# Lumina-Group/libzkp

Hardware: AMD Instinct MI355X
Metric: proofs/sec (whole node) + ms/proof p50, 4096-proof mixed batch (range / equality / membership / improvement) per MI355X (higher is better)
Workload: dtype u32/u64 integer limbs (10x25.5-bit GF(2^255-19), BN254 Fq on 9x29-bit limbs in the MSM loops and 10x26-bit elsewhere, 8x32-bit Fr and scalars mod l, 2x64-bit f128)

## Files before the change

### libzkp_amd/csrc/g16_circuit.h

```cpp
#pragma once
#include <mutex>
#include <array>
#include <map>
#include <vector>
#include <cstring>
#include "g16_steps.h"
#include "sha256_host.h"

namespace zkp {

inline fr fr_pow_words(fr base, const uint32_t e[8]) {
    fr acc = fp_one<FrParams>();
    for (int i = 255; i >= 0; i--) { acc = fp_sq(acc); if ((e[i >> 5] >> (i & 31)) & 1u) acc = fp_mul(acc, base); }
    return acc;
}
inline void put_fr(std::vector<uint32_t>& v, const fr& x) { for (int k = 0; k < 8; k++) v.push_back(x.v[k]); }

struct HostLC { std::map<uint32_t, fr> t; };
struct HostR1CS {
    uint32_t n_inst = 1, n_wit = 0;
    std::vector<std::array<HostLC, 3>> rows;
    std::vector<uint8_t> inst_nwin{1}, wit_nwin;
    uint32_t new_input(uint8_t nwin) { inst_nwin.push_back(nwin); return n_inst++; }
    uint32_t new_witness(uint8_t nwin) { wit_nwin.push_back(nwin); return 0x80000000u | n_wit++; }
// ... 18 lines not shown
}
inline void r1cs_enforce_equal(HostR1CS& cs, const HostLC& a, const HostLC& b) { cs.rows.push_back({lc_sub(a, b), lc_var(VAR_ONE), HostLC{}}); }

inline std::vector<fr> g_mimc_host;
inline std::once_flag g_mimc_once;
inline void ensure_mimc_constants() {
    std::call_once(g_mimc_once, []() {
        for (uint32_t i = 0; i < MIMC_ROUNDS; i++) {
            uint8_t in[23]; memcpy(in, "libzkp_mimc_v1:", 15); for (int k = 0; k < 8; k++) in[15 + k] = (uint8_t)((uint64_t)i >> (8 * k));
            uint8_t h[32]; sha256_host(h, in, 23);
            uint32_t w[8]; memcpy(w, h, 32);
            g_mimc_host.push_back(fp_from_raw<FrParams>(w));
        }
    });
}
inline HostLC r1cs_mimc(HostR1CS& cs, HostLC x) {
    ensure_mimc_constants();
    for (uint32_t i = 0; i < MIMC_ROUNDS; i++) {
        const HostLC t = lc_add(x, lc_scale(lc_var(VAR_ONE), g_mimc_host[i]));
        const uint32_t t2 = r1cs_mul(cs, t, t, G16_NW_FULL);
        const uint32_t t4 = r1cs_mul(cs, lc_var(t2), lc_var(t2), G16_NW_FULL);
        x = lc_var(r1cs_mul(cs, lc_var(t4), t, G16_NW_FULL));
    }
    return x;
}
inline HostR1CS build_equality_r1cs() {
    HostR1CS cs;
    const uint32_t a = cs.new_witness(G16_NW_U64), b = cs.new_witness(G16_NW_U64);
    r1cs_enforce_equal(cs, lc_var(a), lc_var(b));
    const HostLC h = r1cs_mimc(cs, lc_var(a));
    const uint32_t c = cs.new_input(G16_NW_FULL);
    r1cs_enforce_equal(cs, h, lc_var(c));
    return cs;
}
inline HostR1CS build_membership_r1cs() {
    HostR1CS cs;
    const uint32_t v = cs.new_witness(G16_NW_U64);
    const HostLC h = r1cs_mimc(cs, lc_var(v));
    const uint32_t c = cs.new_input(G16_NW_FULL);
    r1cs_enforce_equal(cs, h, lc_var(c));
    std::vector<uint32_t> setv, real, sel;
    for (uint32_t i = 0; i < G16_MAX_SET; i++) setv.push_back(cs.new_input(G16_NW_U64));
    for (uint32_t i = 0; i < G16_MAX_SET; i++) { const uint32_t b = cs.new_input(1); cs.rows.push_back({lc_sub(lc_var(VAR_ONE), lc_var(b)), lc_var(b), HostLC{}}); real.push_back(b); }
    for (uint32_t i = 0; i < G16_MAX_SET; i++) { const uint32_t b = cs.new_witness(1); cs.rows.push_back({lc_sub(lc_var(VAR_ONE), lc_var(b)), lc_var(b), HostLC{}}); sel.push_back(b); }
    HostLC total;
    for (uint32_t i = 0; i < G16_MAX_SET; i++) {
        total = lc_add(total, lc_var(sel[i]));
        const uint32_t p = r1cs_mul(cs, lc_var(sel[i]), lc_sub(lc_var(VAR_ONE), lc_var(real[i])), 1);
        r1cs_enforce_equal(cs, lc_var(p), HostLC{});
    }
    r1cs_enforce_equal(cs, total, lc_var(VAR_ONE));
    HostLC acc;
    for (uint32_t i = 0; i < G16_MAX_SET; i++) acc = lc_add(acc, lc_var(r1cs_mul(cs, lc_var(sel[i]), lc_sub(lc_var(v), lc_var(setv[i])), G16_NW_FULL)));
    r1cs_enforce_equal(cs, acc, HostLC{});
    return cs;
}


struct HostCircuitTables {
    uint32_t n_inst, n_wit, nv, n_rows, m, logm;
    std::vector<uint32_t> ptr[3], col[3], coef[3];
    std::vector<uint32_t> tw, tw_inv, coset, coset_inv, zinv;
};
inline HostCircuitTables build_circuit_tables(const HostR1CS& cs) {
    HostCircuitTables T;
    T.n_inst = cs.n_inst; T.n_wit = cs.n_wit; T.nv = cs.n_inst + cs.n_wit; T.n_rows = (uint32_t)cs.rows.size();
    uint32_t m = 1, lg = 0; while (m < T.n_rows + T.n_inst) { m <<= 1; lg++; }
    T.m = m; T.logm = lg;
    auto colidx = [&](uint32_t v) { return (v & WIT) ? cs.n_inst + (v & ~WIT) : v; };
    for (int q = 0; q < 3; q++) {
        T.ptr[q].push_back(0);
        for (auto& row : cs.rows) {
            for (auto& kv : row[q].t) { T.col[q].push_back(colidx(kv.first)); put_fr(T.coef[q], kv.second); }
            T.ptr[q].push_back((uint32_t)T.col[q].size());
        }
    }
    uint32_t e[8]; for (int i = 0; i < 8; i++) e[i] = FrParams::mod(i);
    e[0] -= 1;
    for (uint32_t s = 0; s < lg; s++) { for (int i = 0; i < 7; i++) e[i] = (e[i] >> 1) | (e[i + 1] << 31); e[7] >>= 1; }
    const fr g = fp_from_u64<FrParams>(5), w = fr_pow_words(g, e);
    const fr winv = fp_inv(w), ginv = fp_inv(g), minv = fp_inv(fp_from_u64<FrParams>(m));
    auto put_fr9 = [](std::vector<uint32_t>& v, const fr& x) { const fr9 y = fr9_from_fr(x); for (int i = 0; i < 9; i++) v.push_back(y.v[i]); };
    fr a = fp_one<FrParams>(), b = a;
    for (uint32_t j = 0; j < m / 2; j++) { put_fr9(T.tw, a); put_fr9(T.tw_inv, b); a = fp_mul(a, w); b = fp_mul(b, winv); }
    a = minv; b = minv;
    for (uint32_t i = 0; i < m; i++) { put_fr9(T.coset, a); put_fr9(T.coset_inv, b); a = fp_mul(a, g); b = fp_mul(b, ginv); }
    fr gm = fp_one<FrParams>(); for (uint32_t i = 0; i < m; i++) gm = fp_mul(gm, g);
    put_fr9(T.zinv, fp_inv(fp_sub(gm, fp_one<FrParams>())));
    return T;
}

}
```

### libzkp_amd/csrc/g16_impl.inc

```

namespace {

struct G16Key {
    bool loaded = false;
    uint32_t n_inst = 0, n_wit = 0, nv = 0, n_rows = 0, m = 0, logm = 0;
    G16Circuit C{};
    std::vector<void*> allocs;
    uint32_t *table_g1 = nullptr, *table_g2 = nullptr;
    G16Radix rx = g16_radix(G16_WBITS_DEFAULT);
    int shared_tables = -1;
    uint64_t table_bytes = 0;
    struct Chunking { DevLayout lay; const uint32_t* corr = nullptr; const uint16_t* scal = nullptr; };
    std::vector<SlotList> targets_g1, targets_g2;
    std::vector<uint16_t> hscal_g1, hscal_g2;
    std::map<uint64_t, Chunking> lays_g1, lays_g2;
    uint64_t win_g1 = 0, win_g2 = 0;
    const uint32_t *init_g1 = nullptr, *init_g2 = nullptr;
    G16Vk vk{}; bool vk_ready = false;
    const uint32_t *vm_kconst = nullptr, *vm_lines = nullptr;
};
struct G16Run {
    void* buf = nullptr; size_t cap = 0; hipStream_t side = nullptr, side2 = nullptr; hipEvent_t ev[4] = {nullptr, nullptr, nullptr, nullptr};
    hipEvent_t last = nullptr; bool used = false;
};
// ... 348 lines not shown
            uint32_t* d_ic_tab = nullptr;
            if ((rc = build_tables<20>(K, ic_pts, &d_ic_tab, false, g16_radix(G16V_WBITS)))) return rc;
            K.vk.gamma = gamma_g2.p; K.vk.delta = delta_g2.p; K.vk.beta = beta_g2.p; K.vk.n_ic = (uint32_t)abc.size(); K.vk.ic = d_ic; K.vk.ic_table = d_ic_tab;
            K.vk.ml_alpha_beta = miller_loop(beta_g2.p, aff_neg(alpha_g1.p));
            std::vector<uint32_t> kc(6 * 20), lines;
            g16_vm_key_constants(beta_g2.p, aff_neg(alpha_g1.p), gamma_g2.p, delta_g2.p, kc.data(), lines);
            if ((rc = dev_upload(K, &K.vm_kconst, kc)) || (rc = dev_upload(K, &K.vm_lines, lines))) return rc;
            K.vk_ready = true;
        }
    }
    K.loaded = true;
    return 0;
}


fr tape_fr(const uint32_t seed[8], uint32_t idx, uint32_t slot) { uint32_t w[16]; tape_draw64(w, seed, idx, slot); return fp_from_wide<FrParams>(w); }

int gpu_scalar_mults(bool g2, const std::vector<fr>& scalars, std::vector<uint8_t>& out_bytes) {
    const uint32_t rows = (uint32_t)scalars.size(), AW = g2 ? 40 : 20, JW = g2 ? G2_JAC_W : G1_JAC_W, PB = g2 ? 128 : 64;
    std::vector<uint32_t> base;
    if (!g2) append_words(base, host_g1_generator()); else append_words(base, host_g2_generator());
    ensure_offsets();
    std::vector<uint32_t> offs;
    if (!g2) { append_words(offs, g_off.o1); append_words(offs, jac_neg(g_off.o1)); } else { append_words(offs, g_off.o2); append_words(offs, jac_neg(g_off.o2)); }
    const G16Radix rx = g16_radix(10);
    std::vector<uint32_t> dig((size_t)rx.digw * rows);
    for (uint32_t i = 0; i < rows; i++) {
        sc raw; fp_to_raw(raw.v, scalars[i]); uint32_t pk[G16_DIGW_MAX]; g16_recode(pk, raw, rx);
        for (uint32_t k = 0; k < rx.digw; k++) dig[(size_t)k * rows + i] = pk[k];
    }
    uint32_t *d_base = nullptr, *d_tab = nullptr, *d_dig = nullptr, *d_part = nullptr, *d_offs = nullptr, *d_sums = nullptr; uint8_t* d_out = nullptr;
    uint16_t* d_meta = nullptr; uint8_t* d_nwin = nullptr; uint32_t* d_steps = nullptr;
    DevScope mem;
    HIP_TRY(mem.alloc(&d_base, AW * 4)); HIP_TRY(mem.alloc(&d_tab, (size_t)rx.slot_ent * g16_table_entry_words(g2, true) * 4 + 64)); HIP_TRY(mem.alloc(&d_dig, dig.size() * 4));
    HIP_TRY(mem.alloc(&d_part, (size_t)JW * 4 * rows)); HIP_TRY(mem.alloc(&d_sums, (size_t)JW * 4 * rows)); HIP_TRY(mem.alloc(&d_offs, offs.size() * 4));
    HIP_TRY(hipMemcpy(d_offs, offs.data(), offs.size() * 4, hipMemcpyHostToDevice)); HIP_TRY(mem.alloc(&d_out, (size_t)PB * rows)); HIP_TRY(mem.alloc(&d_meta, 32)); HIP_TRY(mem.alloc(&d_nwin, 16));
    const uint16_t meta[7] = {0, 0, 0, 0, (uint16_t)rx.nwin, 0, 1};
    const uint8_t nwin = (uint8_t)rx.nwin;
    HIP_TRY(hipMemcpy(d_base, base.data(), AW * 4, hipMemcpyHostToDevice));
    HIP_TRY(hipMemcpy(d_dig, dig.data(), dig.size() * 4, hipMemcpyHostToDevice));
    HIP_TRY(hipMemcpy(d_meta, meta, 14, hipMemcpyHostToDevice)); HIP_TRY(hipMemcpy(d_nwin, &nwin, 1, hipMemcpyHostToDevice));
    uint32_t steps_words = 0;
    {
        MsmLayout L1; L1.slot_base = {0}; L1.slot_nwin = {(uint8_t)rx.nwin}; L1.chunk_begin = {0}; L1.chunk_win0 = {0}; L1.chunk_nwin = {(uint16_t)rx.nwin}; L1.target_chunk_begin = {0, 1};
        std::vector<uint32_t> steps, step0;
        const GatherShape shape{rx.nent, rx.slot_ent, rx.uneven ? 1u : 0u, rx.digw};
        if (!make_gather_steps(L1, nullptr, shape, steps, step0)) return fail(ZKP_HIP_E_UNSUPPORTED, "window tables of more than 2^32 entries");
        steps.insert(steps.end(), step0.begin(), step0.end());
        HIP_TRY(mem.alloc(&d_steps, steps.size() * 4));
        HIP_TRY(hipMemcpy(d_steps, steps.data(), steps.size() * 4, hipMemcpyHostToDevice));
        steps_words = (uint32_t)(steps.size() - step0.size());
    }
    g16_launch_build_table(g2, d_base, 1, d_tab, dev().stream, true, rx);
    MsmView m; m.nwin = rx.nwin; m.nent = rx.nent; m.digw = rx.digw; m.slot_ent = rx.slot_ent; m.uneven = rx.uneven; m.rows = rows; m.nslots = 1; m.nchunks = 1; m.table = d_tab; m.digits = d_dig;
    m.slot_base = d_meta; m.slot_scalar = d_meta + 1; m.slot_nwin = d_nwin; m.chunk_begin = d_meta + 2; m.chunk_win0 = d_meta + 3; m.chunk_nwin = d_meta + 4; m.partial = d_part; m.acc_init = d_offs;
    m.steps = d_steps; m.chunk_step0 = d_steps + steps_words;
    g16_launch_msm(g2, m, dev().stream);
    ReduceView R{}; R.rows = rows; R.ntargets = 1; R.partial = d_part; R.target_chunk_begin = d_meta + 5; R.corr = d_offs + JW;
    g16_launch_sum(g2, R, d_sums, dev().stream);
    g16_launch_serialize(g2, d_sums, rows, d_out, dev().stream);
    out_bytes.resize((size_t)PB * rows);
    HIP_TRY(hipMemcpyAsync(out_bytes.data(), d_out, out_bytes.size(), hipMemcpyDeviceToHost, dev().stream));
    HIP_TRY(hipStreamSynchronize(dev().stream));
    return 0;
}

int generate_key_locked(int kind, const uint8_t* setup_seed, std::vector<uint8_t>& pk, std::vector<uint8_t>& vk) {
    if (kind != G16_EQUALITY && kind != G16_MEMBERSHIP) return fail(ZKP_HIP_E_ARGUMENT, "unknown circuit kind");
    const HostR1CS cs = kind == G16_EQUALITY ? build_equality_r1cs() : build_membership_r1cs();
    const HostCircuitTables T = build_circuit_tables(cs);
    uint32_t seed[8];
    if (setup_seed) memcpy(seed, setup_seed, 32);
    else { std::vector<uint8_t> f; int rc0 = fresh_seeds(f, 1); if (rc0) return rc0; memcpy(seed, f.data(), 32); }
    const char* tagname = kind == G16_EQUALITY ? "equality_mimc" : "membership_mimc";
    uint8_t th[32]; sha256_host(th, (const uint8_t*)tagname, strlen(tagname));
    const uint32_t tag = (uint32_t)th[0] | ((uint32_t)th[1] << 8) | ((uint32_t)th[2] << 16);
    fr tw[5];
    for (uint32_t k = 0; k < 5; k++) { tw[k] = tape_fr(seed, 0x47313601u, 8 * tag + k); if (fp_is_zero(tw[k])) tw[k] = fp_one<FrParams>(); }
    const fr alpha = tw[0], beta = tw[1], gamma = tw[2], delta = tw[3], tau = tw[4];
    const uint32_t m = T.m, nv = T.nv;
    const fr one = fp_one<FrParams>();
    fr taum = one; for (uint32_t i = 0; i < m; i++) taum = fp_mul(taum, tau);
    const fr zt = fp_sub(taum, one), minv = fp_inv(fp_from_u64<FrParams>(m));
    const fr w = fr9_to_fr<FrParams>(ld_fr9_c(T.tw.data(), 1));
    std::vector<fr> lag(m);
    fr wj = one;
    for (uint32_t j = 0; j < m; j++) { lag[j] = fp_mul(fp_mul(fp_mul(zt, minv), wj), fp_inv(fp_sub(tau, wj))); wj = fp_mul(wj, w); }
    std::vector<fr> At(nv, fp_zero<FrParams>()), Bt = At, Ct = At;
    std::vector<fr>* dst[3] = {&At, &Bt, &Ct};
    for (int q = 0; q < 3; q++)
        for (uint32_t j = 0; j < T.n_rows; j++)
            for (uint32_t e = T.ptr[q][j]; e < T.ptr[q][j + 1]; e++)
                (*dst[q])[T.col[q][e]] = fp_add((*dst[q])[T.col[q][e]], fp_mul(ld_fr_c(T.coef[q].data(), e), lag[j]));
    for (uint32_t i = 0; i < T.n_inst; i++) At[i] = fp_add(At[i], lag[T.n_rows + i]);
    const fr ginv = fp_inv(gamma), dinv = fp_inv(delta);
    auto mix = [&](uint32_t k) { return fp_add(fp_add(fp_mul(beta, At[k]), fp_mul(alpha, Bt[k])), Ct[k]); };
    std::vector<fr> s1 = {alpha, beta, delta}, s2 = {beta, gamma, delta};
    for (uint32_t i = 0; i < T.n_inst; i++) s1.push_back(fp_mul(mix(i), ginv));
    for (uint32_t k = 0; k < nv; k++) s1.push_back(At[k]);
    for (uint32_t k = 0; k < nv; k++) s1.push_back(Bt[k]);
    { fr tp = fp_mul(zt, dinv); for (uint32_t i = 0; i + 1 < m; i++) { s1.push_back(tp); tp = fp_mul(tp, tau); } }
    for (uint32_t k = T.n_inst; k < nv; k++) s1.push_back(fp_mul(mix(k), dinv));
    for (uint32_t k = 0; k < nv; k++) s2.push_back(Bt[k]);
    std::vector<uint8_t> b1, b2; int rc;
    if ((rc = gpu_scalar_mults(false, s1, b1)) || (rc = gpu_scalar_mults(true, s2, b2))) return rc;
    auto g1at = [&](size_t i) { return b1.data() + 64 * i; };
    auto g2at = [&](size_t i) { return b2.data() + 128 * i; };
    auto put = [](std::vector<uint8_t>& v, const uint8_t* p, size_t n) { v.insert(v.end(), p, p + n); };
    auto put_len = [](std::vector<uint8_t>& v, uint64_t n) { for (int i = 0; i < 8; i++) v.push_back((uint8_t)(n >> (8 * i))); };
    size_t o_abc = 3, o_a = o_abc + T.n_inst, o_b = o_a + nv, o_h = o_b + nv, o_l = o_h + (m - 1);
    vk.clear();
    put(vk, g1at(0), 64); put(vk, g2at(0), 128); put(vk, g2at(1), 128); put(vk, g2at(2), 128);
    put_len(vk, T.n_inst); put(vk, g1at(o_abc), 64ull * T.n_inst);
    pk = vk;
    put(pk, g1at(1), 64); put(pk, g1at(2), 64);
    put_len(pk, nv); put(pk, g1at(o_a), 64ull * nv);
    put_len(pk, nv); put(pk, g1at(o_b), 64ull * nv);
    put_len(pk, nv); put(pk, g2at(3), 128ull * nv);
    put_len(pk, m - 1); put(pk, g1at(o_h), 64ull * (m - 1));
    put_len(pk, T.n_wit); put(pk, g1at(o_l), 64ull * T.n_wit);
    return load_key_locked(kind, pk.data(), pk.size());
}

int launch_msm_key(bool g2, const G16Radix& rx, const G16Key::Chunking& ch, const uint32_t* table, const uint32_t* acc_init, uint32_t rows, const uint32_t* digits, uint32_t* partial, hipStream_t st) {
    const DevLayout& D = ch.lay; const uint16_t* slot_scalar = ch.scal;
    MsmView m; m.nwin = rx.nwin; m.nent = rx.nent; m.digw = rx.digw; m.slot_ent = rx.slot_ent; m.uneven = rx.uneven; m.rows = rows; m.nslots = D.nslots; m.nchunks = D.nchunks; m.table = table; m.digits = digits;
    m.slot_base = D.slot_base; m.slot_scalar = slot_scalar; m.slot_nwin = D.slot_nwin; m.chunk_begin = D.chunk_begin; m.chunk_win0 = D.chunk_win0; m.chunk_nwin = D.chunk_nwin; m.partial = partial; m.acc_init = acc_init;
    m.steps = D.steps; m.chunk_step0 = D.chunk_step0;
    Device::KProf& K = dev().prof[g2 ? 2 : 1];
    hipEvent_t e1 = nullptr;
    int rc = prof_begin(K, st, &e1);
    if (rc) return rc;
    ZKP_TRACED(g2 ? "k_msm_gather<G2Msm>" : "k_msm_gather<G1Msm>", st, g16_launch_msm(g2, m, st));
    prof_end(K, st, e1, D.adds_per_row * rows);
    return 0;
}


int run_g16(int kind, uint32_t rows, const uint64_t* d_value, const uint64_t* d_set_vals, const uint32_t* d_set_len, const uint8_t* d_seeds,
            uint8_t* d_out, uint64_t stride, hipStream_t st, uint32_t lane = 0) {
    G16Key& K = g16s().key[kind];
    if (!K.loaded) return fail(ZKP_HIP_E_ARGUMENT, "no proving key loaded for this circuit (zkp_hip_groth16_load_key)");
    const uint32_t nsc = g16_nscalars(K.nv, K.m);
    const G16Key::Chunking *c1 = nullptr, *c1c = nullptr, *c2 = nullptr;
    int rc;
    if ((rc = get_chunking(K, false, G16_PART_AB, rows, &c1)) || (rc = get_chunking(K, true, G16_PART_ALL, rows, &c2))) return rc;
    if ((rc = get_chunking(K, false, G16_PART_C, rows, &c1c))) return rc;
    size_t off = 0;
    auto sz = [&](size_t bytes) { size_t o = off; off += align_up(bytes); return o; };
    const size_t W = (size_t)32 * rows;
    const size_t o_z = sz(W * K.nv), o_sd = sz((size_t)K.rx.digw * 4 * rows * nsc), o_rs = sz(W * 2), o_p1 = sz((size_t)c1->lay.nchunks * G1_JAC_W * 4 * rows),
                 o_p1c = sz((size_t)c1c->lay.nchunks * G1_JAC_W * 4 * rows), o_p2 = sz((size_t)c2->lay.nchunks * G2_JAC_W * 4 * rows),
                 o_s1 = sz((size_t)3 * G1_JAC_W * 4 * rows), o_s2 = sz((size_t)G2_JAC_W * 4 * rows), o_t1 = sz((size_t)G16_CPARTS * G1_JAC_W * 4 * rows),
                 o_qe = sz((size_t)2 * 9 * K.m * 4 * rows);
    G16Run& RW = g16s().run[kind][lane & 1u];
    if (off > RW.cap) {
        if (RW.buf) { HIP_TRY(hipDeviceSynchronize()); HIP_TRY(hipFree(RW.buf)); RW.buf = nullptr; RW.cap = 0; }
        HIP_TRY(hipMalloc(&RW.buf, off)); RW.cap = off;
    }
    uint8_t* base = (uint8_t*)RW.buf;
    G16View V{}; V.rx = K.rx; V.rows = rows; V.kind = (uint32_t)kind; V.n_inst = K.n_inst; V.n_wit = K.n_wit; V.nv = K.nv; V.m = K.m;
    V.value = d_value; V.set_vals = d_set_vals; V.set_len = d_set_len; V.seeds = reinterpret_cast<const uint32_t*>(d_seeds); V.mimc_c = g16s().mimc_dev;
    V.z = (uint32_t*)(base + o_z); V.sdig = (uint32_t*)(base + o_sd); V.rs = (uint32_t*)(base + o_rs); V.out = d_out; V.stride = stride;
    V.qap_evals = (uint32_t*)(base + o_qe);
    uint32_t *p1 = (uint32_t*)(base + o_p1), *p1c = (uint32_t*)(base + o_p1c), *p2 = (uint32_t*)(base + o_p2), *s1 = (uint32_t*)(base + o_s1), *s2 = (uint32_t*)(base + o_s2), *t1 = (uint32_t*)(base + o_t1);
    if (!RW.last) {
        for (auto& e : RW.ev) HIP_TRY(hipEventCreateWithFlags(&e, hipEventDisableTiming));
// ... 303 lines not shown
```

### libzkp_amd/csrc/g16_steps.h

```cpp
#pragma once
#include "bn254_g.h"
#include "bn254_fr9.h"
#include "keccak.h"
#include "sc25519.h"

namespace zkp {

struct G16Radix { uint32_t wbits, nwin, nent, digw, nwin_u64, uneven, slot_ent; };
constexpr uint32_t G16_UNEVEN_TOP_ENT = 25088;
ZKP_HD inline G16Radix g16_radix(uint32_t wbits, bool uneven = false) {
    G16Radix r; r.wbits = wbits; r.nwin = (254 + wbits) / wbits; r.nent = 1u << (wbits - 1); r.nwin_u64 = (64 + wbits) / wbits; r.uneven = 0;
    r.slot_ent = r.nwin * r.nent;
    if (uneven && wbits == 14) { r.uneven = 1; r.nwin = 18; r.slot_ent = 18u * r.nent + G16_UNEVEN_TOP_ENT; }
    r.digw = (r.nwin + 1) / 2;
    return r;
}
ZKP_HD inline uint32_t g16_win_bit(const G16Radix& rx, uint32_t w) { return rx.uneven && w == 17 ? 239u : rx.wbits * w; }
ZKP_HD inline uint32_t g16_win_off(const G16Radix& rx, uint32_t w) { return (w + (rx.uneven && w == 17 ? 1u : 0u)) * rx.nent; }
ZKP_HD inline uint32_t g16_win_ent(const G16Radix& rx, uint32_t w) { return !rx.uneven || w < 16 ? rx.nent : w == 16 ? 2u * rx.nent : G16_UNEVEN_TOP_ENT; }
constexpr uint32_t G16_WBITS_DEFAULT = 14, G16_WBITS_KNEE = 13, G16_WBITS_MIN = 8, G16_WBITS_MAX = 15, G16_DIGW_MAX = 16;
static_assert(G16_WBITS_DEFAULT >= G16_WBITS_MIN && G16_WBITS_DEFAULT <= G16_WBITS_MAX, "key-table radix out of range");
ZKP_HD inline void g16_recode_uneven(uint32_t* packed, const sc& raw) {
    uint32_t carry = 0;
    ZKP_UNROLL for (int j = 0; j < 18; j++) {
// ... 69 lines not shown

ZKP_HD inline fr g16_mimc_chain(const G16View& V, uint32_t row, fr x, uint32_t wit0) {
    for (uint32_t i = 0; i < MIMC_ROUNDS; i++) {
        const fr t = fp_add(x, ld_fr_c(V.mimc_c, i));
        const fr t2 = fp_sq(t), t4 = fp_sq(t2);
        x = fp_mul(t4, t);
        if (V.z) { st_fr(V.z, wit0 + 3 * i, row, V.rows, t2); st_fr(V.z, wit0 + 3 * i + 1, row, V.rows, t4); st_fr(V.z, wit0 + 3 * i + 2, row, V.rows, x); }
    }
    return x;
}

ZKP_HD inline void step_g16_witness(const G16View& V, uint32_t row) {
    const uint32_t rows = V.rows;
    const uint64_t val = V.value[row];
    const fr one = fp_one<FrParams>(), zero = fp_zero<FrParams>();
    const fr v = fp_from_u64<FrParams>(val);
    uint8_t* o = V.out + (uint64_t)row * V.stride;
    st_fr(V.z, 0, row, rows, one);
    fr h;
    uint32_t proof_len = 256;
    if (V.kind == G16_EQUALITY) {
        st_fr(V.z, 2, row, rows, v); st_fr(V.z, 3, row, rows, v);
        h = g16_mimc_chain(V, row, v, 4);
        st_fr(V.z, 1, row, rows, h);
        o[0] = 2; o[1] = 2;
    } else {
        const uint32_t len = V.set_len[row];
        const uint64_t* sv = V.set_vals + (size_t)row * G16_MAX_SET;
        const uint32_t w0 = V.n_inst;
        st_fr(V.z, w0, row, rows, v);
        h = g16_mimc_chain(V, row, v, w0 + 1);
        st_fr(V.z, 1, row, rows, h);
        uint32_t pos = 0xffffffffu;
        for (uint32_t i = 0; i < len; i++) if (pos == 0xffffffffu && sv[i] == val) pos = i;
        const uint32_t sel0 = w0 + 1 + 3 * MIMC_ROUNDS;
        for (uint32_t i = 0; i < G16_MAX_SET; i++) {
            const bool real = i < len;
            const fr si = fp_from_u64<FrParams>(real ? sv[i] : 0);
            st_fr(V.z, 2 + i, row, rows, si);
            st_fr(V.z, 2 + G16_MAX_SET + i, row, rows, real ? one : zero);
            const bool sel = i == pos;
            st_fr(V.z, sel0 + i, row, rows, sel ? one : zero);
            st_fr(V.z, sel0 + G16_MAX_SET + i, row, rows, (sel && !real) ? one : zero);
            st_fr(V.z, sel0 + 2 * G16_MAX_SET + i, row, rows, sel ? fp_sub(v, si) : zero);
        }
        o[0] = 2; o[1] = 4;
        proof_len = 4 + 8 * len + 256;
        uint8_t* pl = o + 10;
        pl[0] = (uint8_t)len; pl[1] = (uint8_t)(len >> 8); pl[2] = (uint8_t)(len >> 16); pl[3] = (uint8_t)(len >> 24);
        for (uint32_t i = 0; i < len; i++) for (int k = 0; k < 8; k++) pl[4 + 8 * i + k] = (uint8_t)(sv[i] >> (8 * k));
    }
    for (int k = 0; k < 4; k++) { o[2 + k] = (uint8_t)(proof_len >> (8 * k)); o[6 + k] = (uint8_t)(32u >> (8 * k)); }
    uint32_t hraw[8]; fp_to_raw(hraw, h);
    g16_put_bytes(o + 10 + proof_len, hraw, 8);
    uint32_t seed[8]; ZKP_UNROLL for (int k = 0; k < 8; k++) seed[k] = V.seeds[(size_t)row * 8 + k];
    uint32_t w[16];
    tape_draw64(w, seed, G16_TAPE_IDX, 0); const fr r = fp_from_wide<FrParams>(w);
    tape_draw64(w, seed, G16_TAPE_IDX, 1); const fr s = fp_from_wide<FrParams>(w);
    st_fr_digits(V.sdig, g16_sc_r(V), row, rows, r, V.rx);
    st_fr_digits(V.sdig, g16_sc_s(V), row, rows, s, V.rx);
    st_fr_digits(V.sdig, g16_sc_nrs(V), row, rows, fp_neg(fp_mul(r, s)), V.rx);
    uint32_t* q = V.sdig + (size_t)g16_sc_one(V) * V.rx.digw * rows + row;
    q[0] = 1u; for (uint32_t k = 1; k < V.rx.digw; k++) q[(size_t)k * rows] = 0u;
    fr rr, sr; fp_to_raw(rr.v, r); fp_to_raw(sr.v, s);
    st_fr(V.rs, 0, row, rows, rr); st_fr(V.rs, 1, row, rows, sr);
}
ZKP_HD inline void step_g16_zdigits(const G16View& V, uint32_t k, uint32_t row) {
    st_fr_digits(V.sdig, k, row, V.rows, ld_fr(V.z, k, row, V.rows), V.rx);
}

struct G16Circuit {
    uint32_t n_rows, m, logm;
    const uint32_t *a_ptr, *a_col, *a_coef, *b_ptr, *b_col, *b_coef, *c_ptr, *c_col, *c_coef;
    const uint32_t *tw, *tw_inv;
    const uint32_t *coset, *coset_inv;
    const uint32_t* zinv;
};
ZKP_HD inline fr g16_row_dot(const uint32_t* ptr, const uint32_t* col, const uint32_t* coef, uint32_t r, const uint32_t* z, uint32_t row, uint32_t rows) {
    fr acc = fp_zero<FrParams>();
    for (uint32_t e = ptr[r]; e < ptr[r + 1]; e++) acc = fp_add(acc, fp_mul(ld_fr_c(coef, e), ld_fr(z, col[e], row, rows)));
    return acc;
}
ZKP_HD inline uint32_t g16_bitrev(uint32_t x, uint32_t bits) {
    uint32_t r = 0; for (uint32_t i = 0; i < bits; i++) { r = (r << 1) | (x & 1u); x >>= 1; } return r;
}

struct G16Lds {
    uint32_t* base; uint32_t m;
    ZKP_HD static uint32_t sw(uint32_t e) { return e ^ ((0u - ((e >> 5) & 1u)) & 10u) ^ ((0u - ((e >> 6) & 1u)) & 21u); }
    ZKP_HD fr9 ld(uint32_t e) const { fr9 r; const uint32_t p = sw(e); ZKP_UNROLL for (int k = 0; k < 9; k++) r.v[k] = base[(size_t)k * m + p]; return r; }
    ZKP_HD void st(uint32_t e, const fr9& v) const { const uint32_t p = sw(e); ZKP_UNROLL for (int k = 0; k < 9; k++) base[(size_t)k * m + p] = v.v[k]; }
};
ZKP_HD inline fr9 ld_fr9_c(const uint32_t* p, uint32_t idx) { fr9 r; ZKP_UNROLL for (int k = 0; k < 9; k++) r.v[k] = p[(size_t)idx * 9 + k]; return r; }
ZKP_HD inline fr g16_row_dot_fast(const uint32_t* ptr, const uint32_t* col, const uint32_t* coef, uint32_t r, const uint32_t* z, uint32_t row, uint32_t rows) {
    const fr one = fp_one<FrParams>();
    fr acc = fp_zero<FrParams>();
    for (uint32_t e = ptr[r]; e < ptr[r + 1]; e++) {
        const fr cf = ld_fr_c(coef, e);
        const uint32_t c = col[e];
        bool is_one = true; ZKP_UNROLL for (int k = 0; k < 8; k++) is_one = is_one && cf.v[k] == one.v[k];
        if (c == 0) acc = fp_add(acc, cf);
        else if (is_one) acc = fp_add(acc, ld_fr(z, c, row, rows));
        else acc = fp_add(acc, fp_mul(cf, ld_fr(z, c, row, rows)));
    }
    return acc;
}
ZKP_HD inline void g16_qap_load(const G16View& V, const G16Circuit& C, const G16Lds& L, uint32_t poly, uint32_t row, uint32_t tid, uint32_t nthreads) {
    const uint32_t nc = C.n_rows;
    const uint32_t *ptr = poly == 0 ? C.a_ptr : poly == 1 ? C.b_ptr : C.c_ptr, *col = poly == 0 ? C.a_col : poly == 1 ? C.b_col : C.c_col,
                   *coef = poly == 0 ? C.a_coef : poly == 1 ? C.b_coef : C.c_coef;
    for (uint32_t j = tid; j < C.m; j += nthreads) {
        fr a = fp_zero<FrParams>();
        if (j < nc) a = g16_row_dot_fast(ptr, col, coef, j, V.z, row, V.rows);
        else if (poly == 0 && j < nc + V.n_inst) a = ld_fr(V.z, j - nc, row, V.rows);
        L.st(j, fr9_from_fr(a));
    }
}
ZKP_HD inline void g16_bf_dif(fr9& u, fr9& v, const fr9& w) { const fr9 s = fr9_reduce_weak(fr9_add(u, v)); v = fr9_mul(fr9_sub_k<4>(u, v), w); u = s; }
ZKP_HD inline void g16_bf_dit(fr9& u, fr9& v, const fr9& w) { const fr9 t = fr9_mul(v, w); v = fr9_sub_k<2>(u, t); u = fr9_add(u, t); }
template <bool DIF>
ZKP_HD inline void g16_stage_single(const G16Circuit& C, const G16Lds& L, const uint32_t* tw, uint32_t half, uint32_t tid, uint32_t nthreads) {
    const uint32_t len = 2 * half, tstride = C.m / len;
    for (uint32_t k = tid; k < C.m / 2; k += nthreads) {
        const uint32_t grp = k / half, j = k % half, i0 = grp * len + j, i1 = i0 + half;
        const fr9 w = ld_fr9_c(tw, j * tstride);
        fr9 u = L.ld(i0), v = L.ld(i1);
        if (DIF) g16_bf_dif(u, v, w); else g16_bf_dit(u, v, w);
        L.st(i0, u); L.st(i1, v);
    }
}
template <bool DIF>
ZKP_HD inline void g16_stage_pair(const G16Circuit& C, const G16Lds& L, const uint32_t* tw, uint32_t h, uint32_t tid, uint32_t nthreads) {
    const uint32_t s1 = C.m / (2 * h), s2 = C.m / (4 * h);
    for (uint32_t q = tid; q < C.m / 4; q += nthreads) {
        const uint32_t grp = q / h, j = q % h, e0 = grp * 4 * h + j;
        fr9 x0 = L.ld(e0), x1 = L.ld(e0 + h), x2 = L.ld(e0 + 2 * h), x3 = L.ld(e0 + 3 * h);
        const fr9 wh = ld_fr9_c(tw, j * s1), wa = ld_fr9_c(tw, j * s2), wb = ld_fr9_c(tw, (j + h) * s2);
        if (DIF) { g16_bf_dif(x0, x2, wa); g16_bf_dif(x1, x3, wb); g16_bf_dif(x0, x1, wh); g16_bf_dif(x2, x3, wh); }
        else { g16_bf_dit(x0, x1, wh); g16_bf_dit(x2, x3, wh); g16_bf_dit(x0, x2, wa); g16_bf_dit(x1, x3, wb); }
        L.st(e0, x0); L.st(e0 + h, x1); L.st(e0 + 2 * h, x2); L.st(e0 + 3 * h, x3);
    }
}
template <class Sync> ZKP_HD inline void g16_transform_dif(const G16Circuit& C, const G16Lds& L, const uint32_t* tw, uint32_t tid, uint32_t nthreads, Sync sync) {
    uint32_t half = C.m / 2;
    if (C.logm & 1u) { g16_stage_single<true>(C, L, tw, half, tid, nthreads); sync(); half >>= 1; }
    for (; half >= 2; half >>= 2) { g16_stage_pair<true>(C, L, tw, half / 2, tid, nthreads); sync(); }
}
template <class Sync> ZKP_HD inline void g16_transform_dit(const G16Circuit& C, const G16Lds& L, const uint32_t* tw, uint32_t tid, uint32_t nthreads, Sync sync) {
    uint32_t h = 1;
    for (uint32_t i = 0; i < C.logm / 2; i++, h <<= 2) { g16_stage_pair<false>(C, L, tw, h, tid, nthreads); sync(); }
    if (C.logm & 1u) { g16_stage_single<false>(C, L, tw, C.m / 2, tid, nthreads); sync(); }
}
ZKP_HD inline void g16_scale_bitrev(const G16Circuit& C, const G16Lds& L, const uint32_t* tab, uint32_t tid, uint32_t nthreads) {
    for (uint32_t p = tid; p < C.m; p += nthreads) L.st(p, fr9_mul(L.ld(p), ld_fr9_c(tab, g16_bitrev(p, C.logm))));
}
ZKP_HD inline void g16_spill(const G16Circuit& C, const G16Lds& L, uint32_t* dst, uint32_t tid, uint32_t nthreads) {
    for (uint32_t w = tid; w < 9 * C.m; w += nthreads) dst[w] = L.base[w];
}
ZKP_HD inline fr9 g16_ld_spilled(const uint32_t* src, uint32_t m, uint32_t e) { fr9 r; const uint32_t p = G16Lds::sw(e); ZKP_UNROLL for (int k = 0; k < 9; k++) r.v[k] = src[(size_t)k * m + p]; return r; }
ZKP_HD inline void g16_pointwise(const G16Circuit& C, const G16Lds& L, const uint32_t* ea, const uint32_t* eb, uint32_t tid, uint32_t nthreads) {
    const fr9 zinv = ld_fr9_c(C.zinv, 0);
    for (uint32_t i = tid; i < C.m; i += nthreads)
        L.st(i, fr9_mul(fr9_sub_k<32>(fr9_mul(g16_ld_spilled(ea, C.m, i), g16_ld_spilled(eb, C.m, i)), L.ld(i)), zinv));
}
ZKP_HD inline void g16_store_h_bitrev(const G16View& V, const G16Circuit& C, const G16Lds& L, uint32_t row, uint32_t tid, uint32_t nthreads) {
    for (uint32_t p = tid; p < C.m; p += nthreads) {
        const uint32_t i = g16_bitrev(p, C.logm);
        if (i + 1 < C.m) st_fr_digits(V.sdig, g16_sc_h(V) + i, row, V.rows, fr9_to_fr<FrParams>(fr9_mul(L.ld(p), ld_fr9_c(C.coset_inv, i))), V.rx);
    }
}
template <class Sync>
ZKP_HD inline void g16_qap_proof(const G16View& V, const G16Circuit& C, const G16Lds& L, uint32_t* scratch, uint32_t row, uint32_t tid, uint32_t nthreads, Sync sync) {
    for (uint32_t poly = 0; poly < 3; poly++) {
        g16_qap_load(V, C, L, poly, row, tid, nthreads); sync();
        g16_transform_dif(C, L, C.tw_inv, tid, nthreads, sync);
        g16_scale_bitrev(C, L, C.coset, tid, nthreads); sync();
        g16_transform_dit(C, L, C.tw, tid, nthreads, sync);
        if (poly < 2) { g16_spill(C, L, scratch + (size_t)poly * 9 * C.m, tid, nthreads); sync(); }
    }
    g16_pointwise(C, L, scratch, scratch + (size_t)9 * C.m, tid, nthreads); sync();
    g16_transform_dif(C, L, C.tw_inv, tid, nthreads, sync);
    g16_store_h_bitrev(V, C, L, row, tid, nthreads);
}

#define G1_JAC_W 30
#define G2_JAC_W 60
ZKP_HD inline fq ld_fq_col(const uint32_t* q, uint32_t rows) { fq r; ZKP_UNROLL for (int k = 0; k < 10; k++) r.v[k] = q[(size_t)k * rows]; return r; }
ZKP_HD inline void st_fq_col(uint32_t* q, uint32_t rows, const fq& a) { ZKP_UNROLL for (int k = 0; k < 10; k++) q[(size_t)k * rows] = a.v[k]; }
ZKP_HD inline g1_jac ld_g1_jac(const uint32_t* p, uint32_t idx, uint32_t row, uint32_t rows) {
    const uint32_t* q = p + (size_t)idx * G1_JAC_W * rows + row; const size_t s = (size_t)10 * rows;
    g1_jac r; r.X = ld_fq_col(q, rows); r.Y = ld_fq_col(q + s, rows); r.Z = ld_fq_col(q + 2 * s, rows);
    return r;
}
ZKP_HD inline void st_g1_jac(uint32_t* p, uint32_t idx, uint32_t row, uint32_t rows, const g1_jac& g) {
    uint32_t* q = p + (size_t)idx * G1_JAC_W * rows + row; const size_t s = (size_t)10 * rows;
    st_fq_col(q, rows, g.X); st_fq_col(q + s, rows, g.Y); st_fq_col(q + 2 * s, rows, g.Z);
}
ZKP_HD inline g2_jac ld_g2_jac(const uint32_t* p, uint32_t idx, uint32_t row, uint32_t rows) {
    const uint32_t* q = p + (size_t)idx * G2_JAC_W * rows + row; const size_t s = (size_t)10 * rows;
    g2_jac r;
    r.X.c0 = ld_fq_col(q, rows); r.X.c1 = ld_fq_col(q + s, rows); r.Y.c0 = ld_fq_col(q + 2 * s, rows); r.Y.c1 = ld_fq_col(q + 3 * s, rows);
    r.Z.c0 = ld_fq_col(q + 4 * s, rows); r.Z.c1 = ld_fq_col(q + 5 * s, rows);
    return r;
}
ZKP_HD inline void st_g2_jac(uint32_t* p, uint32_t idx, uint32_t row, uint32_t rows, const g2_jac& g) {
    uint32_t* q = p + (size_t)idx * G2_JAC_W * rows + row; const size_t s = (size_t)10 * rows;
    st_fq_col(q, rows, g.X.c0); st_fq_col(q + s, rows, g.X.c1); st_fq_col(q + 2 * s, rows, g.Y.c0); st_fq_col(q + 3 * s, rows, g.Y.c1);
    st_fq_col(q + 4 * s, rows, g.Z.c0); st_fq_col(q + 5 * s, rows, g.Z.c1);
}
constexpr uint32_t G16_CPARTS = 4;
ZKP_HD inline void step_g16_cparts(const G16View& V, const uint32_t* sum_g1, uint32_t* tmp_g1, uint32_t part, uint32_t row) {
    const uint32_t rows = V.rows, which = part >> 1;
    g1_jac P = ld_g1_jac(sum_g1, which, row, rows);
    const fr k = ld_fr(V.rs, which == 0 ? 1 : 0, row, rows);
    glv_half h1, h2; fr_glv_split(k.v, h1, h2);
    if (part & 1u) P.X = fq_mul(P.X, fq_glv_beta());
    const glv_half& h = (part & 1u) ? h2 : h1;
    st_g1_jac(tmp_g1, part, row, rows, jac_mul_u128_signed(P, h.mag, h.neg));
}
ZKP_HD inline void step_g16_final(const G16View& V, const uint32_t* sum_g1, const uint32_t* sum_g2, const uint32_t* tmp_g1, uint32_t which, uint32_t row) {
    const uint32_t rows = V.rows;
    uint8_t* o = V.out + (uint64_t)row * V.stride;
    uint32_t plen = 0; for (int k = 0; k < 4; k++) plen |= (uint32_t)o[2 + k] << (8 * k);
    uint8_t* pr = o + 10 + plen - 256;
    if (which == 0) {
        uint32_t w1[16]; g1_serialize(w1, ld_g1_jac(sum_g1, 0, row, rows)); g16_put_bytes(pr, w1, 16);
    } else if (which == 1) {
        uint32_t w2[32]; g2_serialize(w2, ld_g2_jac(sum_g2, 0, row, rows)); g16_put_bytes(pr + 64, w2, 32);
    } else {
        g1_jac Cc = ld_g1_jac(sum_g1, 2, row, rows);
        for (uint32_t t = 0; t < G16_CPARTS; t++) Cc = jac_add(Cc, ld_g1_jac(tmp_g1, t, row, rows));
        uint32_t w1[16]; g1_serialize(w1, Cc); g16_put_bytes(pr + 192, w1, 16);
    }
}

}
```

Before: 337,300.

## Fuse coset scaling, spill, pointwise and H store into NTT stage passes

Folds the bit-reversed coset scaling into the first DIT stage, spill to scratch and pointwise product into the last DIT stage, and the H digit store into the final DIF stage via prologue/epilogue functors. This removes several full LDS read/write passes and barriers per polynomial. Twiddle tables are transposed to limb-major layout so lanes read coalesced words, and bit reversal uses a hardware intrinsic on device. Spilled data is now written unswizzled by element index, and the DIT loop structure assumes logm>=4, which adds edge-case risk.

```diff
diff --git a/libzkp_amd/csrc/g16_circuit.h b/libzkp_amd/csrc/g16_circuit.h
--- a/libzkp_amd/csrc/g16_circuit.h
+++ b/libzkp_amd/csrc/g16_circuit.h
@@ -124,7 +124,12 @@
     const fr winv = fp_inv(w), ginv = fp_inv(g), minv = fp_inv(fp_from_u64<FrParams>(m));
     auto put_fr9 = [](std::vector<uint32_t>& v, const fr& x) { const fr9 y = fr9_from_fr(x); for (int i = 0; i < 9; i++) v.push_back(y.v[i]); };
     fr a = fp_one<FrParams>(), b = a;
-    for (uint32_t j = 0; j < m / 2; j++) { put_fr9(T.tw, a); put_fr9(T.tw_inv, b); a = fp_mul(a, w); b = fp_mul(b, winv); }
+    T.tw.assign((size_t)9 * (m / 2), 0); T.tw_inv.assign((size_t)9 * (m / 2), 0);
+    for (uint32_t j = 0; j < m / 2; j++) {
+        const fr9 ya = fr9_from_fr(a), yb = fr9_from_fr(b);
+        for (int i = 0; i < 9; i++) { T.tw[(size_t)i * (m / 2) + j] = ya.v[i]; T.tw_inv[(size_t)i * (m / 2) + j] = yb.v[i]; }
+        a = fp_mul(a, w); b = fp_mul(b, winv);
+    }
     a = minv; b = minv;
     for (uint32_t i = 0; i < m; i++) { put_fr9(T.coset, a); put_fr9(T.coset_inv, b); a = fp_mul(a, g); b = fp_mul(b, ginv); }
     fr gm = fp_one<FrParams>(); for (uint32_t i = 0; i < m; i++) gm = fp_mul(gm, g);
diff --git a/libzkp_amd/csrc/g16_impl.inc b/libzkp_amd/csrc/g16_impl.inc
--- a/libzkp_amd/csrc/g16_impl.inc
+++ b/libzkp_amd/csrc/g16_impl.inc
@@ -454,7 +454,7 @@
     const fr one = fp_one<FrParams>();
     fr taum = one; for (uint32_t i = 0; i < m; i++) taum = fp_mul(taum, tau);
     const fr zt = fp_sub(taum, one), minv = fp_inv(fp_from_u64<FrParams>(m));
-    const fr w = fr9_to_fr<FrParams>(ld_fr9_c(T.tw.data(), 1));
+    const fr w = fr9_to_fr<FrParams>(g16_ld_tw(T.tw.data(), T.m / 2, 1));
     std::vector<fr> lag(m);
     fr wj = one;
     for (uint32_t j = 0; j < m; j++) { lag[j] = fp_mul(fp_mul(fp_mul(zt, minv), wj), fp_inv(fp_sub(tau, wj))); wj = fp_mul(wj, w); }
diff --git a/libzkp_amd/csrc/g16_steps.h b/libzkp_amd/csrc/g16_steps.h
--- a/libzkp_amd/csrc/g16_steps.h
+++ b/libzkp_amd/csrc/g16_steps.h
@@ -175,7 +175,11 @@
     return acc;
 }
 ZKP_HD inline uint32_t g16_bitrev(uint32_t x, uint32_t bits) {
+#if defined(__HIP_DEVICE_COMPILE__)
+    return __builtin_bitreverse32(x) >> (32u - bits);
+#else
     uint32_t r = 0; for (uint32_t i = 0; i < bits; i++) { r = (r << 1) | (x & 1u); x >>= 1; } return r;
+#endif
 }
 
 struct G16Lds {
@@ -185,6 +189,7 @@
     ZKP_HD void st(uint32_t e, const fr9& v) const { const uint32_t p = sw(e); ZKP_UNROLL for (int k = 0; k < 9; k++) base[(size_t)k * m + p] = v.v[k]; }
 };
 ZKP_HD inline fr9 ld_fr9_c(const uint32_t* p, uint32_t idx) { fr9 r; ZKP_UNROLL for (int k = 0; k < 9; k++) r.v[k] = p[(size_t)idx * 9 + k]; return r; }
+ZKP_HD inline fr9 g16_ld_tw(const uint32_t* p, uint32_t half_m, uint32_t idx) { fr9 r; ZKP_UNROLL for (int k = 0; k < 9; k++) r.v[k] = p[(size_t)k * half_m + idx]; return r; }
 ZKP_HD inline fr g16_row_dot_fast(const uint32_t* ptr, const uint32_t* col, const uint32_t* coef, uint32_t r, const uint32_t* z, uint32_t row, uint32_t rows) {
     const fr one = fp_one<FrParams>();
     fr acc = fp_zero<FrParams>();
@@ -211,69 +216,75 @@
 }
 ZKP_HD inline void g16_bf_dif(fr9& u, fr9& v, const fr9& w) { const fr9 s = fr9_reduce_weak(fr9_add(u, v)); v = fr9_mul(fr9_sub_k<4>(u, v), w); u = s; }
 ZKP_HD inline void g16_bf_dit(fr9& u, fr9& v, const fr9& w) { const fr9 t = fr9_mul(v, w); v = fr9_sub_k<2>(u, t); u = fr9_add(u, t); }
-template <bool DIF>
-ZKP_HD inline void g16_stage_single(const G16Circuit& C, const G16Lds& L, const uint32_t* tw, uint32_t half, uint32_t tid, uint32_t nthreads) {
+struct G16Keep { ZKP_HD fr9 operator()(uint32_t, const fr9& x) const { return x; } };
+struct G16Put { G16Lds L; ZKP_HD void operator()(uint32_t e, const fr9& x) const { L.st(e, x); } };
+template <bool DIF, class Epi>
+ZKP_HD inline void g16_stage_single(const G16Circuit& C, const G16Lds& L, const uint32_t* tw, uint32_t half, uint32_t tid, uint32_t nthreads, Epi epi) {
     const uint32_t len = 2 * half, tstride = C.m / len;
     for (uint32_t k = tid; k < C.m / 2; k += nthreads) {
         const uint32_t grp = k / half, j = k % half, i0 = grp * len + j, i1 = i0 + half;
-        const fr9 w = ld_fr9_c(tw, j * tstride);
+        const fr9 w = g16_ld_tw(tw, C.m / 2, j * tstride);
         fr9 u = L.ld(i0), v = L.ld(i1);
         if (DIF) g16_bf_dif(u, v, w); else g16_bf_dit(u, v, w);
-        L.st(i0, u); L.st(i1, v);
-    }
-}
-template <bool DIF>
-ZKP_HD inline void g16_stage_pair(const G16Circuit& C, const G16Lds& L, const uint32_t* tw, uint32_t h, uint32_t tid, uint32_t nthreads) {
-    const uint32_t s1 = C.m / (2 * h), s2 = C.m / (4 * h);
+        epi(i0, u); epi(i1, v);
+    }
+}
+template <bool DIF, class Pro, class Epi>
+ZKP_HD inline void g16_stage_pair(const G16Circuit& C, const G16Lds& L, const uint32_t* tw, uint32_t h, uint32_t tid, uint32_t nthreads, Pro pro, Epi epi) {
+    const uint32_t hm = C.m / 2, s1 = C.m / (2 * h), s2 = C.m / (4 * h);
     for (uint32_t q = tid; q < C.m / 4; q += nthreads) {
         const uint32_t grp = q / h, j = q % h, e0 = grp * 4 * h + j;
-        fr9 x0 = L.ld(e0), x1 = L.ld(e0 + h), x2 = L.ld(e0 + 2 * h), x3 = L.ld(e0 + 3 * h);
-        const fr9 wh = ld_fr9_c(tw, j * s1), wa = ld_fr9_c(tw, j * s2), wb = ld_fr9_c(tw, (j + h) * s2);
+        fr9 x0 = pro(e0, L.ld(e0)), x1 = pro(e0 + h, L.ld(e0 + h)), x2 = pro(e0 + 2 * h, L.ld(e0 + 2 * h)), x3 = pro(e0 + 3 * h, L.ld(e0 + 3 * h));
+        const fr9 wh = g16_ld_tw(tw, hm, j * s1), wa = g16_ld_tw(tw, hm, j * s2), wb = g16_ld_tw(tw, hm, (j + h) * s2);
         if (DIF) { g16_bf_dif(x0, x2, wa); g16_bf_dif(x1, x3, wb); g16_bf_dif(x0, x1, wh); g16_bf_dif(x2, x3, wh); }
         else { g16_bf_dit(x0, x1, wh); g16_bf_dit(x2, x3, wh); g16_bf_dit(x0, x2, wa); g16_bf_dit(x1, x3, wb); }
-        L.st(e0, x0); L.st(e0 + h, x1); L.st(e0 + 2 * h, x2); L.st(e0 + 3 * h, x3);
-    }
-}
-template <class Sync> ZKP_HD inline void g16_transform_dif(const G16Circuit& C, const G16Lds& L, const uint32_t* tw, uint32_t tid, uint32_t nthreads, Sync sync) {
+        epi(e0, x0); epi(e0 + h, x1); epi(e0 + 2 * h, x2); epi(e0 + 3 * h, x3);
+    }
+}
+template <class Sync, class Epi> ZKP_HD inline void g16_transform_dif(const G16Circuit& C, const G16Lds& L, const uint32_t* tw, uint32_t tid, uint32_t nthreads, Sync sync, Epi last) {
+    const G16Keep keep; const G16Put put{L};
     uint32_t half = C.m / 2;
-    if (C.logm & 1u) { g16_stage_single<true>(C, L, tw, half, tid, nthreads); sync(); half >>= 1; }
-    for (; half >= 2; half >>= 2) { g16_stage_pair<true>(C, L, tw, half / 2, tid, nthreads); sync(); }
-}
-template <class Sync> ZKP_HD inline void g16_transform_dit(const G16Circuit& C, const G16Lds& L, const uint32_t* tw, uint32_t tid, uint32_t nthreads, Sync sync) {
-    uint32_t h = 1;
-    for (uint32_t i = 0; i < C.logm / 2; i++, h <<= 2) { g16_stage_pair<false>(C, L, tw, h, tid, nthreads); sync(); }
-    if (C.logm & 1u) { g16_stage_single<false>(C, L, tw, C.m / 2, tid, nthreads); sync(); }
-}
-ZKP_HD inline void g16_scale_bitrev(const G16Circuit& C, const G16Lds& L, const uint32_t* tab, uint32_t tid, uint32_t nthreads) {
-    for (uint32_t p = tid; p < C.m; p += nthreads) L.st(p, fr9_mul(L.ld(p), ld_fr9_c(tab, g16_bitrev(p, C.logm))));
-}
-ZKP_HD inline void g16_spill(const G16Circuit& C, const G16Lds& L, uint32_t* dst, uint32_t tid, uint32_t nthreads) {
-    for (uint32_t w = tid; w < 9 * C.m; w += nthreads) dst[w] = L.base[w];
-}
-ZKP_HD inline fr9 g16_ld_spilled(const uint32_t* src, uint32_t m, uint32_t e) { fr9 r; const uint32_t p = G16Lds::sw(e); ZKP_UNROLL for (int k = 0; k < 9; k++) r.v[k] = src[(size_t)k * m + p]; return r; }
-ZKP_HD inline void g16_pointwise(const G16Circuit& C, const G16Lds& L, const uint32_t* ea, const uint32_t* eb, uint32_t tid, uint32_t nthreads) {
-    const fr9 zinv = ld_fr9_c(C.zinv, 0);
-    for (uint32_t i = tid; i < C.m; i += nthreads)
-        L.st(i, fr9_mul(fr9_sub_k<32>(fr9_mul(g16_ld_spilled(ea, C.m, i), g16_ld_spilled(eb, C.m, i)), L.ld(i)), zinv));
-}
-ZKP_HD inline void g16_store_h_bitrev(const G16View& V, const G16Circuit& C, const G16Lds& L, uint32_t row, uint32_t tid, uint32_t nthreads) {
-    for (uint32_t p = tid; p < C.m; p += nthreads) {
-        const uint32_t i = g16_bitrev(p, C.logm);
-        if (i + 1 < C.m) st_fr_digits(V.sdig, g16_sc_h(V) + i, row, V.rows, fr9_to_fr<FrParams>(fr9_mul(L.ld(p), ld_fr9_c(C.coset_inv, i))), V.rx);
+    if (C.logm & 1u) { g16_stage_single<true>(C, L, tw, half, tid, nthreads, put); sync(); half >>= 1; }
+    for (; half > 2; half >>= 2) { g16_stage_pair<true>(C, L, tw, half / 2, tid, nthreads, keep, put); sync(); }
+    g16_stage_pair<true>(C, L, tw, 1, tid, nthreads, keep, last);
+}
+template <class Sync, class Pro, class Epi> ZKP_HD inline void g16_transform_dit(const G16Circuit& C, const G16Lds& L, const uint32_t* tw, uint32_t tid, uint32_t nthreads, Sync sync, Pro first, Epi last) {
+    const G16Keep keep; const G16Put put{L};
+    g16_stage_pair<false>(C, L, tw, 1, tid, nthreads, first, put); sync();
+    uint32_t h = 4;
+    for (uint32_t i = 1; i + 1 < C.logm / 2; i++, h <<= 2) { g16_stage_pair<false>(C, L, tw, h, tid, nthreads, keep, put); sync(); }
+    if (C.logm & 1u) {
+        g16_stage_pair<false>(C, L, tw, h, tid, nthreads, keep, put); sync();
+        g16_stage_single<false>(C, L, tw, C.m / 2, tid, nthreads, last);
+    } else {
+        g16_stage_pair<false>(C, L, tw, h, tid, nthreads, keep, last);
     }
 }
 template <class Sync>
 ZKP_HD inline void g16_qap_proof(const G16View& V, const G16Circuit& C, const G16Lds& L, uint32_t* scratch, uint32_t row, uint32_t tid, uint32_t nthreads, Sync sync) {
-    for (uint32_t poly = 0; poly < 3; poly++) {
+    const uint32_t m = C.m, logm = C.logm;
+    const G16Put put{L};
+    const auto scale = [&](uint32_t p, const fr9& x) { return fr9_mul(x, ld_fr9_c(C.coset, g16_bitrev(p, logm))); };
+    for (uint32_t poly = 0; poly < 2; poly++) {
+        uint32_t* dst = scratch + (size_t)poly * 9 * m;
+        const auto park = [&](uint32_t e, const fr9& x) { ZKP_UNROLL for (int k = 0; k < 9; k++) dst[(size_t)k * m + e] = x.v[k]; };
         g16_qap_load(V, C, L, poly, row, tid, nthreads); sync();
-        g16_transform_dif(C, L, C.tw_inv, tid, nthreads, sync);
-        g16_scale_bitrev(C, L, C.coset, tid, nthreads); sync();
-        g16_transform_dit(C, L, C.tw, tid, nthreads, sync);
-        if (poly < 2) { g16_spill(C, L, scratch + (size_t)poly * 9 * C.m, tid, nthreads); sync(); }
-    }
-    g16_pointwise(C, L, scratch, scratch + (size_t)9 * C.m, tid, nthreads); sync();
-    g16_transform_dif(C, L, C.tw_inv, tid, nthreads, sync);
-    g16_store_h_bitrev(V, C, L, row, tid, nthreads);
+        g16_transform_dif(C, L, C.tw_inv, tid, nthreads, sync, put); sync();
+        g16_transform_dit(C, L, C.tw, tid, nthreads, sync, scale, park); sync();
+    }
+    const fr9 zinv = ld_fr9_c(C.zinv, 0);
+    const auto pointwise = [&](uint32_t e, const fr9& x) {
+        fr9 a, b; ZKP_UNROLL for (int k = 0; k < 9; k++) { a.v[k] = scratch[(size_t)k * m + e]; b.v[k] = scratch[(size_t)(9 + k) * m + e]; }
+        L.st(e, fr9_mul(fr9_sub_k<32>(fr9_mul(a, b), x), zinv));
+    };
+    g16_qap_load(V, C, L, 2, row, tid, nthreads); sync();
+    g16_transform_dif(C, L, C.tw_inv, tid, nthreads, sync, put); sync();
+    g16_transform_dit(C, L, C.tw, tid, nthreads, sync, scale, pointwise); sync();
+    const auto store_h = [&](uint32_t p, const fr9& x) {
+        const uint32_t i = g16_bitrev(p, logm);
+        if (i + 1 < m) st_fr_digits(V.sdig, g16_sc_h(V) + i, row, V.rows, fr9_to_fr<FrParams>(fr9_mul(x, ld_fr9_c(C.coset_inv, i))), V.rx);
+    };
+    g16_transform_dif(C, L, C.tw_inv, tid, nthreads, sync, store_h);
 }
 
 #define G1_JAC_W 30
```

Result: no change. 336,500 (median of 3 runs) (-0.3%).
